# bobocode/lmono

Measured on AMD Instinct MI355X. Metric: KITTI HDL-64 scans/sec (scanRegistration + laserOdometry), higher is better.
Workload: dtype f32 features / f64 solve

## Files before the change

lmono_amd/csrc/batch.hpp:

```cpp
#pragma once
#include "common.hpp"

namespace lmono {

constexpr int kCornerTable = 16384;
constexpr int kSurfTable = 131072;
constexpr unsigned long long kEmptyKey = ~0ull;

struct __attribute__((aligned(16))) GridCell {
    unsigned long long key;
    int start;
    int cnt;
};

struct BatchView {
    const float4 *in;
    const int64_t *off;
    int n_scans;
    int scan0;
    int n_lines;
    int n_limit;
    int has_grid;
    float min_range;
    float4 *cloud;
    float *curv;
    int8_t *label;
    uint8_t *gap;
    int8_t *ring_tmp;
    int *seg_hist;
    int *scan_ends;
    int *scan_half;
    float *scan_ori;
    int *ring_begin;
    int *n_cloud;
    int *status;
    int *sel_sharp;
    int *sel_sharp_n;
    int *sel_flat;
    int *sel_flat_n;
    float4 *lf_tmp;
    int *lf_n;
    int *sel_todo;
    int *li_todo;
    int *vox_todo;
    float4 *sharp;
    float4 *less_sharp;
    float4 *flat;
    float4 *less_flat;
    int *feat_n;
    int *line_first_ge;
    int *line_last_le;
    GridCell *cg_cell;
    GridCell *sg_cell;
    float4 *cg_pts;
    float4 *sg_pts;
    float4 *lbc_pts;
    float4 *lbs_pts;
    int *lb_start;
    float4 *lb_elev;
    int *grid_mask;
};

}
```

lmono_amd/csrc/frontend.hip:

```cpp
#include "batch.hpp"
#include "ring_decide.hpp"
#include "sel_rounds.hpp"
#include "vox_runs.hpp"

namespace lmono {

__device__ __forceinline__ int ring_of(float angle, int n_lines, bool &discard)
{
    int id = 0;
    discard = false;
    if (n_lines == 16) {
        id = (int)((double)((angle + 15.0f) / 2.0f) + 0.5);
        if (id > n_lines - 1 || id < 0) discard = true;
    } else if (n_lines == 32) {
        id = (int)(((double)angle + 92.0 / 3.0) * 3.0 / 4.0);
        if (id > n_lines - 1 || id < 0) discard = true;
    } else {
        if ((double)angle >= -8.83)
            id = (int)((double)(2.0f - angle) * 3.0 + 0.5);
        else
            id = n_lines / 2 + (int)((-8.83 - (double)angle) * 2.0 + 0.5);
        if ((double)angle > 2.0 || (double)angle < -24.33 || id > 50 || id < 0) discard = true;
    }
    return id;
}

__device__ __forceinline__ bool point_valid(const float4 &p, float mr2)
{
    return isfinite(p.x) & isfinite(p.y) & isfinite(p.z) & !(p.x * p.x + p.y * p.y + p.z * p.z < mr2);
}

constexpr int kRtT = 256, kRtW = kRtT / 64;
constexpr int kRtSeg = 1024;
constexpr int kRtTile = kRtSeg * kRtW;

__device__ __forceinline__ int ring_scan_points(const BatchView &b, int s, int64_t off)
{
    const int n = (int)(b.off[s + 1] - off);
    return b.n_limit > 0 && b.n_limit < n ? b.n_limit : n;
}

__global__ __launch_bounds__(256) void k_ring_ends(BatchView b)
{
    const int s = b.scan0 + blockIdx.x;
    const int64_t off = b.off[s];
    const int n = ring_scan_points(b, s, off);
    const float4 *in = b.in + off;
    const int tid = threadIdx.x, lane = tid & 63;
    __shared__ int s_first;
    if (tid == 0) s_first = INT_MAX;
    __syncthreads();
    const float mr2 = b.min_range * b.min_range;
    for (int c0 = 0; c0 < n; c0 += 256) {
        const int i = c0 + tid;
        int lf = (i < n && point_valid(in[i], mr2)) ? i : INT_MAX;
        lf = wave_min_i(lf);
        if (lane == 0 && lf != INT_MAX) atomicMin(&s_first, lf);
        __syncthreads();
        const int f = s_first;
        __syncthreads();
        if (f != INT_MAX) break;
    }
    if (s_first == INT_MAX) {
        int *rb = b.ring_begin + s * 65;
        if (tid < 65) rb[tid] = 0;
        if (tid == 0) { b.n_cloud[s] = 0; b.scan_ends[s * 2] = -1; b.scan_ends[s * 2 + 1] = -1; b.scan_half[s] = INT_MAX; }
        return;
    }
    if (tid == 0) {
        const float4 p0 = in[s_first];
        b.scan_ori[s * 4] = (float)(-det_atan2((double)p0.y, (double)p0.x));
        float ux, uy;
        ring_start_dir(p0.x, p0.y, ux, uy);
        b.scan_ori[s * 4 + 2] = ux; b.scan_ori[s * 4 + 3] = uy;
        b.scan_ends[s * 2] = s_first; b.scan_ends[s * 2 + 1] = -1;
        b.scan_half[s] = INT_MAX;
    }
}

__global__ __launch_bounds__(kRtT) void k_ring_tag(BatchView b)
{
    const int s = b.scan0 + blockIdx.y;
    const int64_t off = b.off[s];
// ... 87 lines not shown
        for (int u = 0; u < 8; u++) t[u] = h[(size_t)(g + u) * 64];
#pragma unroll
        for (int u = 0; u < 8; u++) { h[(size_t)(g + u) * 64] = run; run += t[u]; }
    }
    for (; g < nseg; g++) { const int t = h[(size_t)g * 64]; h[(size_t)g * 64] = run; run += t; }
    int incl = run;
#pragma unroll
    for (int o = 1; o < 64; o <<= 1) { const int v = __shfl_up(incl, o); if (r >= o) incl += v; }
    int *rb = b.ring_begin + s * 65;
    rb[r] = incl - run;
    if (r == 63) { rb[64] = incl; b.n_cloud[s] = incl; }
}

__global__ __launch_bounds__(kRtT) void k_ring_scatter(BatchView b)
{
    const int s = b.scan0 + blockIdx.y;
    const int64_t off = b.off[s];
    const int n = ring_scan_points(b, s, off);
    const int t0 = blockIdx.x * kRtTile;
    if (t0 >= n || b.scan_ends[s * 2] < 0) return;
    const float4 *in = b.in + off;
    const int tid = threadIdx.x, lane = tid & 63, wave = tid >> 6;
    __shared__ int s_pos[kRtW][64];
    __shared__ double s_atan[17];
    if (tid < 17) s_atan[tid] = kAtanTab[tid];
    const int c_lo = t0 + wave * kRtSeg, c_hi = min(c_lo + kRtSeg, n);
    s_pos[wave][lane] = c_lo < n ? b.seg_hist[((size_t)(off >> 10) + (size_t)s + (size_t)(c_lo >> 10)) * 64 + lane] + b.ring_begin[s * 65 + lane] : 0;
    __syncthreads();
    const float startOri = b.scan_ori[s * 4], endOri = b.scan_ori[s * 4 + 1];
    const int half = b.scan_half[s];
    for (int r0 = c_lo; r0 < c_hi; r0 += 256) {
        int id[4], dstp[4];
        signed char idb[4];
#pragma unroll
        for (int q = 0; q < 4; q++) { const int i = r0 + 64 * q + lane; idb[q] = b.ring_tmp[off + min(i, c_hi - 1)]; }
#pragma unroll
        for (int q = 0; q < 4; q++) { const int i = r0 + 64 * q + lane; id[q] = (i < c_hi) ? (int)idb[q] : -1; }
        float4 pq[4];
#pragma unroll
        for (int q = 0; q < 4; q++) {
            const int i = r0 + 64 * q + lane;
            pq[q] = make_float4(0.f, 0.f, 0.f, 0.f);
            if (id[q] >= 0) pq[q] = in[i];
        }
#pragma unroll
        for (int q = 0; q < 4; q++) {
            dstp[q] = 0;
            unsigned long long rem = __ballot(id[q] >= 0);
            while (rem) {
                const int src = __ffsll((long long)rem) - 1;
                const int k = __shfl(id[q], src);
                const unsigned long long m = __ballot(id[q] == k);
                int base = 0;
                if (lane == src) { base = s_pos[wave][k]; s_pos[wave][k] = base + __popcll(m); }
                base = __shfl(base, src);
                if (id[q] == k) dstp[q] = base + __popcll(m & ((1ull << lane) - 1ull));
                rem &= ~m;
            }
        }
#pragma unroll
        for (int q = 0; q < 4; q++) {
            const int i = r0 + 64 * q + lane;
            if (id[q] >= 0) {
                const float4 p = pq[q];
                float ori = (float)(-det_atan2((double)p.y, (double)p.x, s_atan));
                if (i <= half) {
                    if ((double)ori < (double)startOri - LM_PI / 2.0) ori = (float)((double)ori + 2.0 * LM_PI);
                    else if ((double)ori > (double)startOri + LM_PI * 3.0 / 2.0) ori = (float)((double)ori - 2.0 * LM_PI);
                } else {
                    ori = (float)((double)ori + 2.0 * LM_PI);
                    if ((double)ori < (double)endOri - LM_PI * 3.0 / 2.0) ori = (float)((double)ori + 2.0 * LM_PI);
                    else if ((double)ori > (double)endOri + LM_PI / 2.0) ori = (float)((double)ori - 2.0 * LM_PI);
                }
                const float relTime = (ori - startOri) / (endOri - startOri);
                const float inten = (float)((double)id[q] + 0.1 * (double)relTime);
                b.cloud[off + dstp[q]] = make_float4(p.x, p.y, p.z, inten);
            }
        }
    }
}

constexpr int kCurvTile = 1024;

__global__ __launch_bounds__(256) void k_curvature(BatchView b)
{
    const int s = b.scan0 + blockIdx.y;
    const int n = b.n_cloud[s];
    const int t0 = blockIdx.x * kCurvTile;
    if (t0 >= n) return;
    const int64_t off = b.off[s];
    const float4 *c = b.cloud + off;
    __shared__ float sx[kCurvTile + 10], sy[kCurvTile + 10], sz[kCurvTile + 10];
    for (int k = threadIdx.x; k < kCurvTile + 10; k += 256) {
        const int i = t0 - 5 + k;
        float4 p = make_float4(0.f, 0.f, 0.f, 0.f);
        if (i >= 0 && i < n) p = c[i];
        sx[k] = p.x; sy[k] = p.y; sz[k] = p.z;
    }
    __syncthreads();
    for (int k = threadIdx.x; k < kCurvTile; k += 256) {
        const int i = t0 + k;
        if (i >= n) break;
        const int q = k + 5;
        float cv = 0.f;
        if (i >= 5 && i < n - 5) {
            const float dx = sx[q - 5] + sx[q - 4] + sx[q - 3] + sx[q - 2] + sx[q - 1] - 10 * sx[q] + sx[q + 1] + sx[q + 2] + sx[q + 3] + sx[q + 4] + sx[q + 5];
            const float dy = sy[q - 5] + sy[q - 4] + sy[q - 3] + sy[q - 2] + sy[q - 1] - 10 * sy[q] + sy[q + 1] + sy[q + 2] + sy[q + 3] + sy[q + 4] + sy[q + 5];
            const float dz = sz[q - 5] + sz[q - 4] + sz[q - 3] + sz[q - 2] + sz[q - 1] - 10 * sz[q] + sz[q + 1] + sz[q + 2] + sz[q + 3] + sz[q + 4] + sz[q + 5];
            cv = dx * dx + dy * dy + dz * dz;
        }
        b.curv[off + i] = cv;
        unsigned char g = 0;
        if (i + 1 < n) {
            const float gx = sx[q + 1] - sx[q], gy = sy[q + 1] - sy[q], gz = sz[q + 1] - sz[q];
            g = ((double)(gx * gx + gy * gy + gz * gz) > 0.05) ? 1 : 0;
        }
        b.gap[off + i] = g;
    }
}

constexpr int kSelMaxPerLane = (kRingCap / 6 + 1 + 63) / 64;

__device__ __forceinline__ unsigned int select_lo(int idx, unsigned int reach) { return ((unsigned int)idx << 8) | reach; }

__device__ __forceinline__ unsigned int lane_before(unsigned int v) { return (unsigned int)__builtin_amdgcn_update_dpp(0, (int)v, 0x138, 0xf, 0xf, true); }
__device__ __forceinline__ unsigned int lane_behind(unsigned int v) { return (unsigned int)__builtin_amdgcn_update_dpp(0, (int)v, 0x130, 0xf, 0xf, true); }

constexpr int kSelScratch = 64 * 8;

template <int M>
__device__ __forceinline__ void select_sector(int lane, int j, int sp, int slen, int rbeg, const float *curv, unsigned char *picked,
                                              signed char *label, const unsigned long long *gap, int *sel_sh, int *sel_sh_n, int *sel_fl, int *sel_fl_n,
                                              unsigned int *scratch)
{
    unsigned int kh[M], kl[M];
    unsigned int dead = 0, big = 0, small = 0;
    const int e0 = lane * M;
    unsigned int gwin;
    {
        const int jw = sp + min(e0, slen - 1) - 5;
        const unsigned long long wa = gap[jw >> 6], wb = gap[(jw >> 6) + 1];
        const int sh = jw & 63;
        gwin = (unsigned int)((wa >> sh) | (sh ? wb << (64 - sh) : 0ull));
    }
#pragma unroll
    for (int m = 0; m < M; m++) {
        const int e = e0 + m;
        const bool in = e < slen;
        const int i = sp + min(e, slen - 1);
        const float c = curv[i];
        const unsigned int win = gwin >> m;
        const int lf = min(5, __ffs((int)((win >> 5) | 32u)) - 1);
        const int lb = min(5, __clz((int)((win & 31u) << 27)));
        kh[m] = in ? __float_as_uint(c) : 0u; kl[m] = in ? select_lo(i, (unsigned int)(lf | (lb << 4))) : 0u;
        dead |= (unsigned int)(!in | (picked[i] != 0)) << m;
        big |= (unsigned int)(in & (c >= 0.1f)) << m;
        small |= (unsigned int)(in & (c < 0.1f)) << m;
    }
    int largest = 0;
    unsigned int members = 0u;
    {
        unsigned int live = big & ~dead;
        while (__ballot(live != 0u)) {
            unsigned int x[M + 2 * kSelReach];
#pragma unroll
            for (int m = 0; m < M; m++) x[m + kSelReach] = kh[m] & (unsigned int)((int)(live << (31 - m)) >> 31);
#pragma unroll
            for (int d = 0; d < kSelReach; d++) {
                x[d] = lane_before(x[M + d]);
                x[M + kSelReach + d] = lane_behind(x[kSelReach + d]);
            }
            const unsigned int w = sel_winners<M>(x, gwin);
            members |= w;
            live &= ~sel_deaths<M>(sel_window<M>(lane_before(w), w, lane_behind(w)), gwin);
        }
    }
    int n_mem = 0;
#pragma unroll
    for (int m = 0; m < M; m++) n_mem += __popcll(__ballot((members >> m) & 1u));
    unsigned int top = members;
    if (n_mem > 64) {
        const unsigned int best = sel_lane_best<M>(members, kh);
        int above = 0;
        for (int t = 0; t < 64; t++) above += (unsigned int)__builtin_amdgcn_readlane((int)best, t) > best ? 1 : 0;
        top = sel_keep_from<M>(members, kh, wave_min_u32_uniform(above < kSelSharpMax ? best : ~0u));
    }
    int n_top = 0;
#pragma unroll
    for (int m = 0; m < M; m++) {
        const bool is = (top >> m) & 1u;
        const unsigned long long mk = __ballot(is);
        const int pos = n_top + __popcll(mk & ((1ull << lane) - 1ull));
        if (is && pos < 64) { scratch[2 * pos] = kh[m]; scratch[2 * pos + 1] = kl[m]; }
        n_top += __popcll(mk);
    }
    const bool ranked = n_top <= 64;
    if (ranked) {
        __builtin_amdgcn_wave_barrier();
        unsigned int ch = 0u, cl = 0u;
        if (lane < n_top) { ch = scratch[2 * lane]; cl = scratch[2 * lane + 1]; }
        __builtin_amdgcn_wave_barrier();
        int rank = 0;
        for (int t = 0; t < n_top; t++) {
            const unsigned int th = (unsigned int)__builtin_amdgcn_readlane((int)ch, t), tl = (unsigned int)__builtin_amdgcn_readlane((int)cl, t);
            rank += sel_key_above(th, tl, ch, cl) ? 1 : 0;
        }
        if (lane < n_top && rank < kSelSharpMax) {
            const int pind = (int)(cl >> 8), lf = sel_lf(cl), lb = sel_lb(cl);
            sel_sh[j * 20 + rank] = rbeg + pind; label[pind] = rank < 2 ? 2 : 1;
#pragma unroll
            for (int o = 0; o <= 2 * kSelReach; o++) picked[pind - lb + min(o, lf + lb)] = 1;
        }
        largest = n_mem;
        __builtin_amdgcn_wave_barrier();
#pragma unroll
        for (int m = 0; m < M; m++) dead |= (unsigned int)(picked[sp + min(e0 + m, slen - 1)] != 0) << m;
    }
    while (!ranked) {
        const unsigned int live = big & ~dead;
        unsigned int bh = 0u, bl = 0u;
#pragma unroll
        for (int m = 0; m < M; m++) {
            const unsigned int h = kh[m] & (unsigned int)((int)(live << (31 - m)) >> 31);
            const bool t = h >= bh;
            bh = t ? h : bh; bl = t ? kl[m] : bl;
        }
        const unsigned int mh = wave_max_u32_uniform(bh);
        if (mh == 0u) break;
        const unsigned long long who = __ballot(bh == mh);
        unsigned int lo;
        if ((who & (who - 1ull)) == 0ull) lo = (unsigned int)__builtin_amdgcn_readlane((int)bl, __ffsll((long long)who) - 1);
        else lo = wave_max_u32_uniform(bh == mh ? bl : 0u);
        const int pind = (int)(lo >> 8), lf = (int)(lo & 15u), lb = (int)((lo >> 4) & 15u);
        largest++;
        if (largest > 20) break;
        if (lane == 0) { sel_sh[j * 20 + largest - 1] = rbeg + pind; label[pind] = largest <= 2 ? 2 : 1; }
        if (lane <= lf + lb) picked[pind - lb + lane] = 1;
        dead |= sel_hit_bits<M>(pind - lb - sp - e0, lb + lf);
    }
    if (lane == 0) sel_sh_n[j] = largest > 20 ? 20 : largest;
    int smallest = 0;
    while (true) {
        const unsigned int live = small & ~dead;
        unsigned int bh = ~0u, bl = ~0u;
#pragma unroll
        for (int m = 0; m < M; m++) {
            const unsigned int h = kh[m] | ~(unsigned int)((int)(live << (31 - m)) >> 31);
            const bool t = h < bh;
            bh = t ? h : bh; bl = t ? kl[m] : bl;
        }
        const unsigned int mh = wave_min_u32_uniform(bh);
        if (mh == ~0u) break;
        const unsigned long long who = __ballot(bh == mh);
        unsigned int lo;
        if ((who & (who - 1ull)) == 0ull) lo = (unsigned int)__builtin_amdgcn_readlane((int)bl, __ffsll((long long)who) - 1);
        else lo = wave_min_u32_uniform(bh == mh ? bl : ~0u);
        const int pind = (int)(lo >> 8), lf = (int)(lo & 15u), lb = (int)((lo >> 4) & 15u);
        if (lane == 0) { label[pind] = -1; sel_fl[j * 4 + smallest] = rbeg + pind; }
        smallest++;
        if (smallest >= 4) break;
        if (lane <= lf + lb) picked[pind - lb + lane] = 1;
        dead |= sel_hit_bits<M>(pind - lb - sp - e0, lb + lf);
    }
    if (lane == 0) sel_fl_n[j] = smallest;
}

__device__ __noinline__ void select_sector_wide(int lane, int j, int sp, int slen, int rbeg, const float *curv, unsigned char *picked,
                                                signed char *label, const unsigned long long *gap, int *sel_sh, int *sel_sh_n, int *sel_fl, int *sel_fl_n,
                                                unsigned int *scratch)
{
    select_sector<kSelMaxPerLane>(lane, j, sp, slen, rbeg, curv, picked, label, gap, sel_sh, sel_sh_n, sel_fl, sel_fl_n, scratch);
}

__device__ __forceinline__ int uni(int v) { return __builtin_amdgcn_readfirstlane(v); }
__device__ __forceinline__ long long uni64(long long v)
{
    const unsigned int lo = (unsigned int)__builtin_amdgcn_readfirstlane((int)(unsigned int)v), hi = (unsigned int)__builtin_amdgcn_readfirstlane((int)(unsigned int)((unsigned long long)v >> 32));
    return (long long)(((unsigned long long)hi << 32) | lo);
}
template <typename T> __device__ __forceinline__ T *uni_ptr(T *p)
{
    typedef __attribute__((address_space(1))) T GT;
    return (T *)(GT *)uni64((long long)p);
}

__host__ __device__ constexpr int sel_slice_bytes(int cap) { return 2 * cap; }

__device__ __forceinline__ void select_ring(BatchView &b, int r, int s, int lane, unsigned char *smem_w, int cap, bool may_defer, unsigned int *scratch)
{
    r = uni(r); s = uni(s);
    const int64_t off = uni64(b.off[s]);
    const int *rb = b.ring_begin + s * 65;
    const int rbeg = uni(rb[r]), rend = uni(rb[r + 1]), len = rend - rbeg;
    const int S = rbeg + 5, E = rend - 6;
    int *sel_sh = uni_ptr(b.sel_sharp + (size_t)((s * 64 + r) * kSectors) * 20);
    int *sel_sh_n = uni_ptr(b.sel_sharp_n + (s * 64 + r) * kSectors);
    int *sel_fl = uni_ptr(b.sel_flat + (size_t)((s * 64 + r) * kSectors) * 4);
    int *sel_fl_n = uni_ptr(b.sel_flat_n + (s * 64 + r) * kSectors);
    if (E - S < 6 || len > kRingCap) {
        if (lane < kSectors) { sel_sh_n[lane] = 0; sel_fl_n[lane] = 0; }
        if (lane == 0 && len > kRingCap) atomicOr(&b.status[s], kStatusRingOverflow);
        for (int i = lane; i < len; i += 64) b.label[off + rbeg + i] = 0;
        return;
    }
    if (len > cap) {
        if (may_defer && lane == 0) b.sel_todo[1 + atomicAdd(&b.sel_todo[0], 1)] = (s << 6) | r;
        return;
    }
    unsigned char *picked = smem_w;
    signed char *label = uni_ptr((signed char *)(b.label + off + rbeg));
    const float *curv = uni_ptr(b.curv + off + rbeg);
    const int span = E - S;
    unsigned long long *gap = (unsigned long long *)(picked + cap);
    for (int i0 = 0; i0 < len + 64; i0 += 64) {
        const int i = i0 + lane;
        unsigned char g = 0;
        if (i < len) { picked[i] = 0; label[i] = 0; g = b.gap[off + rbeg + i]; }
        const unsigned long long mk = __ballot(g != 0);
        if (lane == 0) gap[i0 >> 6] = mk;
    }
    __builtin_amdgcn_wave_barrier();
    for (int j = 0; j < kSectors; j++) {
        const int sp = 5 + span * j / 6;
        const int ep = 5 + span * (j + 1) / 6 - 1;
        const int slen = ep - sp + 1;
        if (slen <= 5 * 64) select_sector<5>(lane, j, sp, slen, rbeg, curv, picked, label, gap, sel_sh, sel_sh_n, sel_fl, sel_fl_n, scratch);
        else if (slen <= 6 * 64) select_sector<6>(lane, j, sp, slen, rbeg, curv, picked, label, gap, sel_sh, sel_sh_n, sel_fl, sel_fl_n, scratch);
        else select_sector_wide(lane, j, sp, slen, rbeg, curv, picked, label, gap, sel_sh, sel_sh_n, sel_fl, sel_fl_n, scratch);
    }
}

constexpr int kSelSmallCap = 2304, kSelBigGrid = 128;

__global__ __launch_bounds__(256, 8) void k_select(BatchView b, int cap, int from_list)
{
    const int lane = threadIdx.x & 63, wave = __builtin_amdgcn_readfirstlane((int)(threadIdx.x >> 6));
    extern __shared__ __align__(16) unsigned char smem[];
    unsigned char *smem_w = smem + wave * sel_slice_bytes(cap);
    unsigned int *scratch = (unsigned int *)(smem + 4 * sel_slice_bytes(cap) + wave * kSelScratch);
    if (!from_list) {
        select_ring(b, blockIdx.x * 4 + wave, b.scan0 + blockIdx.y, lane, smem_w, cap, true, scratch);
    } else {
        const int n_todo = b.sel_todo[0];
        for (int k = blockIdx.x * 4 + wave; k < n_todo; k += gridDim.x * 4) {
            const int e = b.sel_todo[1 + k];
            select_ring(b, e & 63, e >> 6, lane, smem_w, cap, false, scratch);
        }
    }
}

constexpr int kVoxBucketSegsBig = 1024;
constexpr int kVoxSmallSlots = 9, kVoxSmallBits = 11;
constexpr int kVoxBigSlots = kRingCap / 256, kVoxBigBits = 12;
constexpr int kVoxBigGrid = 512;
template <int kSlots, int kBits, bool kSmall>
struct VoxCfg {
    static constexpr int kSegCap = kSmall ? 256 * kSlots : kVoxBucketSegsBig;
    static constexpr int kHistBytes = (1 << kBits) * 2 > kSegCap * 2 ? (1 << kBits) * 2 : kSegCap * 2;
    static constexpr int kKeyBytes = kSmall ? kSegCap * 4 + kSegCap * 2 + kSegCap * 2 + kHistBytes : kRingCap * 8;
    static constexpr int kLds = kKeyBytes + 1024 + (kSlots * 4 + 2) * 8 + kSlots * 4 * 4;
};
static_assert(256 * kVoxSmallSlots <= 4096, "a first index of the small instantiation has 12 bits");
static_assert((1 << kVoxSmallBits) == 2048, "the small instantiation's counters are one uint4 per thread");
constexpr int kVoxLdsSmall = VoxCfg<kVoxSmallSlots, kVoxSmallBits, true>::kLds;
constexpr int kVoxLdsBig = VoxCfg<kVoxBigSlots, kVoxBigBits, false>::kLds;
static_assert(2 * kVoxBucketSegsBig * 8 + (1 << kVoxBigBits) * 4 <= kRingCap * 8, "bucket sort scratch must fit the key region");
#ifdef LMONO_VOX_PROF
#define VT(i) { if (blockIdx.x == 20 && blockIdx.y == 3 && threadIdx.x == 0) vt[i] = clock64(); }
#else
#define VT(i)
#endif

template <int kCtrl, int kRowMask>
__device__ __forceinline__ float dpp_mov_f32(float v, float ident)
{
    return __uint_as_float(dpp_mov_u32<kCtrl, kRowMask>(__float_as_uint(v), __float_as_uint(ident)));
}
__device__ __forceinline__ float wave_min_f(float v)
{
    v = fminf(v, dpp_mov_f32<0x111, 0xf>(v, FLT_MAX));
    v = fminf(v, dpp_mov_f32<0x112, 0xf>(v, FLT_MAX));
    v = fminf(v, dpp_mov_f32<0x114, 0xf>(v, FLT_MAX));
    v = fminf(v, dpp_mov_f32<0x118, 0xf>(v, FLT_MAX));
    v = fminf(v, dpp_mov_f32<0x142, 0xa>(v, FLT_MAX));
    v = fminf(v, dpp_mov_f32<0x143, 0xc>(v, FLT_MAX));
    return __uint_as_float((unsigned int)__builtin_amdgcn_readlane((int)__float_as_uint(v), 63));
}
__device__ __forceinline__ float wave_max_f(float v)
{
    v = fmaxf(v, dpp_mov_f32<0x111, 0xf>(v, -FLT_MAX));
    v = fmaxf(v, dpp_mov_f32<0x112, 0xf>(v, -FLT_MAX));
    v = fmaxf(v, dpp_mov_f32<0x114, 0xf>(v, -FLT_MAX));
    v = fmaxf(v, dpp_mov_f32<0x118, 0xf>(v, -FLT_MAX));
    v = fmaxf(v, dpp_mov_f32<0x142, 0xa>(v, -FLT_MAX));
    v = fmaxf(v, dpp_mov_f32<0x143, 0xc>(v, -FLT_MAX));
    return __uint_as_float((unsigned int)__builtin_amdgcn_readlane((int)__float_as_uint(v), 63));
}
__device__ __forceinline__ int wave_scan_incl_dpp(int v)
{
    v += (int)dpp_mov_u32<0x111, 0xf>((unsigned int)v, 0u);
    v += (int)dpp_mov_u32<0x112, 0xf>((unsigned int)v, 0u);
    v += (int)dpp_mov_u32<0x114, 0xf>((unsigned int)v, 0u);
    v += (int)dpp_mov_u32<0x118, 0xf>((unsigned int)v, 0u);
    v += (int)dpp_mov_u32<0x142, 0xa>((unsigned int)v, 0u);
    v += (int)dpp_mov_u32<0x143, 0xc>((unsigned int)v, 0u);
    return v;
}

template <int kVoxSlots, int kVoxBucketBits, bool kSmall>
__device__ __forceinline__ void voxel_ring(BatchView &b, int r, int s);

// ... 527 lines not shown
```

lmono_amd/csrc/lidar_abi.hip:

```cpp
#pragma once
constexpr int kListGrid = 256;

struct lmono_scan_batch {
    lmono_ctx *ctx = nullptr;
    int n_cap = 0;
    int64_t pts_cap = 0;
    int n_scans = 0;
    int64_t total = 0;
    int max_pts = 0;
    bool registered = false;
    bool grid_built = false;
    std::vector<int64_t> off_h;
    bool validation_pending = false;
    DevOwner mem;
    BatchView v{};
    int64_t *off_d = nullptr;
    float *in_owned = nullptr;
    hipEvent_t staged_ev = nullptr, in_free_ev = nullptr;
    int64_t staged_points = -1;
    std::vector<int> feat_h;
    int chains_cap = 0;
    double *state = nullptr, *incr = nullptr, *poses = nullptr, *xq = nullptr;
    int *corr = nullptr, *lm_info = nullptr, *corr_pair = nullptr, *seed = nullptr;
    float4 *crec = nullptr, *crec_pair = nullptr;
    float4 *lmrec = nullptr;
    size_t lmrec_cap = 0;
    unsigned int *wl = nullptr;
    size_t wl_cap = 0;
    double *ws = nullptr, *resid_d = nullptr;
    int *rstat = nullptr;
    unsigned int *rcount = nullptr;
    hipEvent_t rep_ev[2] = { nullptr, nullptr };
    lmono_boundary_report brep{};
    std::vector<double> resid_h;
    std::vector<int> rerun_h;
    int last_chains = 0, last_lead = 0, last_first = 0;
};

extern "C" void lmono_batch_destroy(lmono_scan_batch *b)
{
    if (!b) return;
    b->mem.clear();
    for (auto &e : b->rep_ev) if (e) (void)hipEventDestroy(e);
    if (b->staged_ev) (void)hipEventDestroy(b->staged_ev);
    if (b->in_free_ev) (void)hipEventDestroy(b->in_free_ev);
    delete b;
}

extern "C" lmono_scan_batch *lmono_batch_create(lmono_ctx *c, int n_cap, int64_t pts_cap)
{
    if (!c || n_cap <= 0 || pts_cap <= 0) return nullptr;
    if (hipSetDevice(c->device) != hipSuccess) return nullptr;
    lmono_scan_batch *b = new lmono_scan_batch();
    b->ctx = c; b->n_cap = n_cap; b->pts_cap = pts_cap;
    BatchView &v = b->v;
    const size_t T = (size_t)pts_cap, N = (size_t)n_cap;
    DevOwner &m = b->mem;
    bool ok = true;
    ok = ok && m.alloc(b->off_d, N + 1);
    ok = ok && m.alloc(v.cloud, T) && m.alloc(v.curv, T) && m.alloc(v.label, T) && m.alloc(v.gap, T);
    ok = ok && m.alloc(v.ring_tmp, T);
    ok = ok && m.alloc(v.seg_hist, ((T >> 10) + N + 1) * 64) && m.alloc(v.scan_ends, N * 2) && m.alloc(v.scan_half, N) && m.alloc(v.scan_ori, N * 4);
    ok = ok && m.alloc(v.ring_begin, N * 65) && m.alloc(v.n_cloud, N) && m.alloc(v.status, N);
    ok = ok && m.alloc(v.sel_sharp, N * 64 * 6 * 20) && m.alloc(v.sel_sharp_n, N * 64 * 6);
    ok = ok && m.alloc(v.sel_flat, N * 64 * 6 * 4) && m.alloc(v.sel_flat_n, N * 64 * 6);
    ok = ok && m.alloc(v.lf_tmp, T) && m.alloc(v.lf_n, N * 64) && m.alloc(v.vox_todo, N * 64 + 1) && m.alloc(v.sel_todo, N * 64 + 1) && m.alloc(v.li_todo, N * 2 + 1);
    ok = ok && m.alloc(v.sharp, N * kMaxSharp) && m.alloc(v.less_sharp, N * kMaxLessSharp);
    ok = ok && m.alloc(v.flat, N * kMaxFlat) && m.alloc(v.less_flat, T);
    ok = ok && m.alloc(v.feat_n, N * 4) && m.alloc(v.line_first_ge, N * 2 * 66) && m.alloc(v.line_last_le, N * 2 * 66);
    ok = ok && m.alloc(v.cg_cell, N * kCornerTable) && m.alloc(v.sg_cell, N * kSurfTable);
    ok = ok && m.alloc(v.cg_pts, N * kMaxLessSharp) && m.alloc(v.sg_pts, T) && m.alloc(v.grid_mask, N * 2);
    ok = ok && m.alloc(v.lbc_pts, N * kMaxLessSharp + kLbPad) && m.alloc(v.lbs_pts, T + kLbPad) && m.alloc(v.lb_start, N * 2 * (kLineKeys + 1)) && m.alloc(v.lb_elev, N * 2 * 66);
    ok = ok && m.alloc(b->incr, N * 7) && m.alloc(b->poses, N * 7) && m.alloc(b->xq, 8);
    ok = ok && m.alloc(b->corr_pair, (size_t)kMaxQueries * 4) && m.alloc(b->crec_pair, (size_t)kMaxQueries * 4);
    if (!ok) {
        c->err = "lmono_batch_create: hipMalloc failed";
        lmono_batch_destroy(b);
        return nullptr;
    }
    v.off = b->off_d;
    return b;
}

static int rings_used(int n_lines) { return n_lines == 64 ? 51 : n_lines; }

static int scanreg_launch(lmono_ctx *c, lmono_scan_batch *b, int scan0, int n_scans, int64_t max_pts, int n_limit = 0)
{
    BatchView v = b->v;
    v.scan0 = scan0; v.n_limit = n_limit;
    hipStream_t st = c->stream;
    c->ev = c->next_set();
    if (!c->ev) { c->err = "hipEventCreate failed"; return LMONO_ENODEV; }
    c->sets[c->n_sets - 1].reg = true;
    HIP_TRY(c, hipMemsetAsync(v.status + scan0, 0, sizeof(int) * n_scans, st));
    HIP_TRY(c, hipMemsetAsync(v.vox_todo, 0, sizeof(int), st));
    HIP_TRY(c, hipMemsetAsync(v.sel_todo, 0, sizeof(int), st));
    HIP_TRY(c, hipMemsetAsync(v.li_todo, 0, sizeof(int), st));
    HIP_TRY(c, hipEventRecord(c->ev[0], st));
    const int rt_tiles = (int)((max_pts + kRtTile - 1) / kRtTile);
    hipLaunchKernelGGL(k_ring_ends, dim3(n_scans), dim3(256), 0, st, v);
    if (rt_tiles > 0) hipLaunchKernelGGL(k_ring_tag, dim3(rt_tiles, n_scans), dim3(kRtT), 0, st, v);
    hipLaunchKernelGGL(k_ring_offsets, dim3(n_scans), dim3(64), 0, st, v);
    if (rt_tiles > 0) hipLaunchKernelGGL(k_ring_scatter, dim3(rt_tiles, n_scans), dim3(kRtT), 0, st, v);
    HIP_TRY(c, hipEventRecord(c->ev[1], st));
    const int tiles = (int)((max_pts + kCurvTile - 1) / kCurvTile);
    if (tiles > 0) hipLaunchKernelGGL(k_curvature, dim3(tiles, n_scans), dim3(256), 0, st, v);
    HIP_TRY(c, hipEventRecord(c->ev[2], st));
    const int n_rings = rings_used(b->v.n_lines);
    HIP_TRY(c, hipMemsetAsync(v.sel_sharp_n + (size_t)scan0 * 64 * 6, 0, sizeof(int) * (size_t)n_scans * 64 * 6, st));
    HIP_TRY(c, hipMemsetAsync(v.sel_flat_n + (size_t)scan0 * 64 * 6, 0, sizeof(int) * (size_t)n_scans * 64 * 6, st));
    HIP_TRY(c, hipMemsetAsync(v.lf_n + (size_t)scan0 * 64, 0, sizeof(int) * (size_t)n_scans * 64, st));
    hipLaunchKernelGGL(k_select, dim3((n_rings + 3) / 4, n_scans), dim3(256), 4 * sel_slice_bytes(kSelSmallCap) + 4 * kSelScratch, st, v, kSelSmallCap, 0);
    hipLaunchKernelGGL(k_select, dim3(kSelBigGrid), dim3(256), 4 * sel_slice_bytes(kRingCap) + 4 * kSelScratch, st, v, (int)kRingCap, 1);
    HIP_TRY(c, hipEventRecord(c->ev[3], st));
    hipLaunchKernelGGL((k_voxel<kVoxSmallSlots, kVoxSmallBits, true>), dim3(n_rings, n_scans), dim3(256), kVoxLdsSmall, st, v);
    hipLaunchKernelGGL((k_voxel<kVoxBigSlots, kVoxBigBits, false>), dim3(kVoxBigGrid), dim3(256), kVoxLdsBig, st, v);
    HIP_TRY(c, hipEventRecord(c->ev[4], st));
    hipLaunchKernelGGL(k_compact_index, dim3(n_scans), dim3(kLiT), kLiLdsHalf, st, v);
    HIP_TRY(c, hipEventRecord(c->ev[5], st));
#ifdef LMONO_DIAG_SEARCH
    if (c->opt[LMONO_OPT_CORR_TILE] != 3) {
        hipLaunchKernelGGL(k_grid_build, dim3(n_scans, 1 + kGridPar), dim3(1024), kGridLds, st, v);
        b->grid_built = true; v.has_grid = 1; b->v.has_grid = 1;
    }
#endif
    HIP_TRY(c, hipEventRecord(c->ev[6], st));
    hipLaunchKernelGGL(k_line_index<false>, dim3(kLiBigGrid), dim3(kLiT), kLiLdsFull, st, v);
    HIP_TRY(c, hipEventRecord(c->ev[7], st));
    return check_launch(c, "scanreg kernels");
}

extern "C" int lmono_scanreg_batch(lmono_ctx *c, lmono_scan_batch *b, const float *xyzi_d, const int64_t *offsets_h,
                                   int n_scans, int n_lines, float min_range);

static int batch_own_input(lmono_ctx *c, lmono_scan_batch *b)
{
    if (b->in_owned || b->mem.alloc(b->in_owned, (size_t)b->pts_cap * 4)) return LMONO_OK;
    const hipError_t e = hipGetLastError();
    c->err = std::string("hipMalloc(&q, (size_t)(b->pts_cap > 0 ? b->pts_cap : 1) * 16): ") + hipGetErrorString(e);
    return e == hipErrorOutOfMemory ? LMONO_ENOMEM : LMONO_ENODEV;
}

extern "C" int lmono_scanreg_batch_h(lmono_ctx *c, lmono_scan_batch *b, const float *xyzi_h, const int64_t *offsets_h,
                                     int n_scans, int n_lines, float min_range)
{
    if (!c || !b || !xyzi_h || !offsets_h || n_scans <= 0) return LMONO_EINVAL;
    if (offsets_h[0] != 0) { c->err = "offsets must start at 0"; return LMONO_EINVAL; }
    const int64_t total = offsets_h[n_scans];
    if (total < 0 || total > b->pts_cap) { c->err = "batch: too many points"; return LMONO_ECAPACITY; }
    HIP_TRY(c, hipSetDevice(c->device));
    if (int rc = batch_own_input(c, b)) return rc;
    if (total > 0) {
        HIP_TRY(c, hipMemcpyAsync(b->in_owned, xyzi_h, (size_t)total * 16, hipMemcpyHostToDevice, c->stream));
        HIP_TRY(c, hipStreamSynchronize(c->stream));
    }
    return lmono_scanreg_batch(c, b, b->in_owned, offsets_h, n_scans, n_lines, min_range);
}

extern "C" int lmono_scanreg_batch(lmono_ctx *c, lmono_scan_batch *b, const float *xyzi_d, const int64_t *offsets_h,
                                   int n_scans, int n_lines, float min_range)
{
    if (!c || !b || !xyzi_d || !offsets_h || n_scans <= 0) return LMONO_EINVAL;
    if (n_lines != 16 && n_lines != 32 && n_lines != 64) { c->err = "n_lines must be 16, 32 or 64"; return LMONO_EINVAL; }
    if (n_scans > b->n_cap) { c->err = "batch: too many scans"; return LMONO_ECAPACITY; }
    int64_t max_pts = 0;
    for (int s = 0; s < n_scans; s++) {
        const int64_t m = offsets_h[s + 1] - offsets_h[s];
        if (m < 0 || m > INT_MAX / 2) { c->err = "bad offsets"; return LMONO_EINVAL; }
        max_pts = m > max_pts ? m : max_pts;
    }
    const int64_t total = offsets_h[n_scans] - offsets_h[0];
    if (offsets_h[0] != 0) { c->err = "offsets must start at 0"; return LMONO_EINVAL; }
    if (total > b->pts_cap) { c->err = "batch: too many points"; return LMONO_ECAPACITY; }
    HIP_TRY(c, hipSetDevice(c->device));
    b->off_h.assign(offsets_h, offsets_h + n_scans + 1);
    b->n_scans = n_scans; b->total = total; b->max_pts = (int)max_pts; b->registered = false; b->grid_built = false;
    b->feat_h.clear();
    BatchView &v = b->v;
    v.in = (const float4 *)xyzi_d; v.n_scans = n_scans; v.scan0 = 0; v.n_lines = n_lines; v.min_range = min_range; v.has_grid = 0;
    HIP_TRY(c, hipMemcpyAsync(b->off_d, b->off_h.data(), sizeof(int64_t) * (n_scans + 1), hipMemcpyHostToDevice, c->stream));
    int rc = scanreg_launch(c, b, 0, n_scans, max_pts);
    if (rc) return rc;
    b->registered = true;
    return LMONO_OK;
}

extern "C" int lmono_batch_stage_h(lmono_ctx *c, lmono_scan_batch *b, const float *xyzi_h, int64_t total_points)
{
    if (!c || !b || !xyzi_h || total_points < 0) return LMONO_EINVAL;
// ... 33 lines not shown

extern "C" int lmono_timing_read(lmono_ctx *c, double *ms, int cap, int *n_scanreg_calls, int *n_odom_calls)
{
    if (!c || !ms) return LMONO_EINVAL;
    HIP_TRY(c, hipStreamSynchronize(c->stream));
    double sum[13] = { 0 };
    int nr = 0, no = 0;
    float t;
    for (int i = 0; i < c->n_sets; i++) {
        const EvSet &s = c->sets[i];
        if (s.reg) {
            nr++;
            if (hipEventElapsedTime(&t, s.e[0], s.e[7]) == hipSuccess) sum[0] += t;
            for (int k = 0; k < 7; k++)
                if (hipEventElapsedTime(&t, s.e[k], s.e[k + 1]) == hipSuccess) sum[2 + k] += t;
        }
        if (s.odom) {
            no++;
            if (hipEventElapsedTime(&t, s.e[8], s.e[9]) == hipSuccess) sum[1] += t;
            for (int k = 0; k + 2 < s.n_kev; k += 3) {
                if (k + 2 >= (int)s.kev.size()) break;
                if (hipEventElapsedTime(&t, s.kev[k], s.kev[k + 1]) == hipSuccess) sum[9] += t;
                if (hipEventElapsedTime(&t, s.kev[k + 1], s.kev[k + 2]) == hipSuccess) sum[10] += t;
                sum[11] += 1.0;
            }
        }
    }
    {
        unsigned long long st[40] = { 0 };
        HIP_TRY(c, hipMemcpy(st, c->stats_d, 320, hipMemcpyDeviceToHost));
        sum[12] = (double)st[0];
        for (int i = 1; i < 40 && 12 + i < cap; i++) ms[12 + i] = (double)st[i];
    }
    for (int i = 0; i < cap && i < 13; i++) ms[i] = sum[i];
    if (n_scanreg_calls) *n_scanreg_calls = nr;
    if (n_odom_calls) *n_odom_calls = no;
    return LMONO_OK;
}

extern "C" int lmono_batch_counts(lmono_ctx *c, lmono_scan_batch *b, int32_t *counts_h)
{
    if (!c || !b || !counts_h || !b->registered) return LMONO_EINVAL;
    const int n = b->n_scans;
    std::vector<int> nc(n), fn(n * 4), stt(n);
    HIP_TRY(c, hipStreamSynchronize(c->stream));
    HIP_TRY(c, hipMemcpy(nc.data(), b->v.n_cloud, sizeof(int) * n, hipMemcpyDeviceToHost));
    HIP_TRY(c, hipMemcpy(fn.data(), b->v.feat_n, sizeof(int) * n * 4, hipMemcpyDeviceToHost));
    HIP_TRY(c, hipMemcpy(stt.data(), b->v.status, sizeof(int) * n, hipMemcpyDeviceToHost));
    for (int s = 0; s < n; s++) {
        counts_h[6 * s] = nc[s];
        for (int k = 0; k < 4; k++) counts_h[6 * s + 1 + k] = fn[4 * s + k];
        counts_h[6 * s + 5] = stt[s];
    }
    return LMONO_OK;
}

extern "C" int lmono_batch_get_cloud(lmono_ctx *c, lmono_scan_batch *b, int scan, int which, float *out_h, int cap)
{
    if (!c || !b || !out_h || !b->registered || scan < 0 || scan >= b->n_scans || which < 0 || which > 4) return LMONO_EINVAL;
    HIP_TRY(c, hipStreamSynchronize(c->stream));
    int n = 0;
    const float4 *src = nullptr;
    int fn[4];
    HIP_TRY(c, hipMemcpy(fn, b->v.feat_n + scan * 4, sizeof(fn), hipMemcpyDeviceToHost));
    switch (which) {
    case 0: HIP_TRY(c, hipMemcpy(&n, b->v.n_cloud + scan, sizeof(int), hipMemcpyDeviceToHost)); src = b->v.cloud + b->off_h[scan]; break;
    case 1: n = fn[0]; src = b->v.sharp + (size_t)scan * kMaxSharp; break;
    case 2: n = fn[1]; src = b->v.less_sharp + (size_t)scan * kMaxLessSharp; break;
    case 3: n = fn[2]; src = b->v.flat + (size_t)scan * kMaxFlat; break;
    default: n = fn[3]; src = b->v.less_flat + b->off_h[scan]; break;
    }
    if (n > cap) { c->err = "get_cloud: output capacity too small"; return LMONO_ECAPACITY; }
    if (n > 0) HIP_TRY(c, hipMemcpy(out_h, src, sizeof(float4) * n, hipMemcpyDeviceToHost));
    return n;
}

extern "C" int lmono_batch_get_curvature(lmono_ctx *c, lmono_scan_batch *b, int scan, float *curv_h, int32_t *label_h, int cap)
{
    if (!c || !b || !b->registered || scan < 0 || scan >= b->n_scans) return LMONO_EINVAL;
    HIP_TRY(c, hipStreamSynchronize(c->stream));
    int n = 0;
    HIP_TRY(c, hipMemcpy(&n, b->v.n_cloud + scan, sizeof(int), hipMemcpyDeviceToHost));
    if (n > cap) { c->err = "get_curvature: output capacity too small"; return LMONO_ECAPACITY; }
    if (curv_h && n > 0) HIP_TRY(c, hipMemcpy(curv_h, b->v.curv + b->off_h[scan], sizeof(float) * n, hipMemcpyDeviceToHost));
    if (label_h && n > 0) {
        std::vector<int8_t> tmp(n);
        HIP_TRY(c, hipMemcpy(tmp.data(), b->v.label + b->off_h[scan], n, hipMemcpyDeviceToHost));
        for (int i = 0; i < n; i++) label_h[i] = tmp[i];
    }
    return n;
}

static int ensure_odom_ws(lmono_ctx *c, lmono_scan_batch *b, int n_chains)
{
    DevOwner &m = b->mem;
    const size_t lmrec_need = (size_t)(n_chains > b->chains_cap ? n_chains : b->chains_cap) * (4 - c->lm_planes) * kMaxQueries;
    if (lmrec_need > b->lmrec_cap) {
        if (!m.alloc(b->lmrec, lmrec_need)) { c->err = "odometry workspace: hipMalloc failed"; return LMONO_ENOMEM; }
        b->lmrec_cap = lmrec_need;
    }
    if (n_chains <= b->chains_cap) return LMONO_OK;
    bool ok = m.alloc(b->state, (size_t)n_chains * 8) && m.alloc(b->corr, (size_t)n_chains * kMaxQueries * 4) &&
              m.alloc(b->lm_info, (size_t)n_chains * 4) && m.alloc(b->crec, (size_t)n_chains * kMaxQueries * 4) &&
              m.alloc(b->seed, (size_t)n_chains * kMaxQueries) && m.alloc(b->wl, 8 * ((size_t)n_chains * kMaxQueries + 1)) &&
              m.alloc(b->ws, (size_t)n_chains * 8) && m.alloc(b->resid_d, (size_t)n_chains) && m.alloc(b->rstat, (size_t)n_chains * 4) &&
              m.alloc(b->rcount, (size_t)n_chains + 2);
    if (!ok) { c->err = "odometry workspace: hipMalloc failed"; return LMONO_ENOMEM; }
    b->chains_cap = n_chains;
    return LMONO_OK;
}

static int ensure_grid(lmono_ctx *c, lmono_scan_batch *b)
{
    if (b->grid_built) return LMONO_OK;
#ifdef LMONO_DIAG_SEARCH
    hipLaunchKernelGGL(k_grid_build, dim3(b->n_scans, 1 + kGridPar), dim3(1024), kGridLds, c->stream, b->v);
    int rc = check_launch(c, "k_grid_build");
    if (rc) return rc;
    b->grid_built = true; b->v.has_grid = 1;
    return LMONO_OK;
#else
    c->err = "the hash-grid searches exist in the diagnostic build only (-DLMONO_DIAG_SEARCH)";
    return LMONO_EINVAL;
#endif
}

struct GroupFork {
    lmono_ctx *c; int G, g_own; bool forked = false;
    GroupFork(lmono_ctx *c_, int G_, int g_own_) : c(c_), G(G_), g_own(g_own_) {}
    int fork()
    {
        if (G <= 1) return LMONO_OK;
        for (int g = g_own; g < G; g++)
            if (!c->gstream[g]) {
                int lo = 0, hi = 0;
                if (c->odom_prio && hipDeviceGetStreamPriorityRange(&lo, &hi) == hipSuccess) HIP_TRY(c, hipStreamCreateWithPriority(&c->gstream[g], hipStreamNonBlocking, hi));
                else HIP_TRY(c, hipStreamCreateWithFlags(&c->gstream[g], hipStreamNonBlocking));
            }
        for (int g = 0; g <= G && g < 9; g++) if (!c->gev[g]) HIP_TRY(c, hipEventCreateWithFlags(&c->gev[g], hipEventDisableTiming));
        HIP_TRY(c, hipEventRecord(c->gev[0], c->stream));
        forked = true;
        for (int g = g_own; g < G; g++) HIP_TRY(c, hipStreamWaitEvent(c->gstream[g], c->gev[0], 0));
        return LMONO_OK;
    }
    int join()
    {
        if (!forked) return LMONO_OK;
        forked = false;
        int rc = LMONO_OK;
        for (int g = g_own; g < G; g++) {
            if (hipEventRecord(c->gev[g + 1], c->gstream[g]) != hipSuccess || hipStreamWaitEvent(c->stream, c->gev[g + 1], 0) != hipSuccess) {
                (void)hipStreamSynchronize(c->gstream[g]);
                c->err = "odometry: joining a chain-group stream failed"; rc = LMONO_ENODEV;
            }
        }
        return rc;
    }
    ~GroupFork() { (void)join(); }
};

static int odom_groups(const lmono_ctx *c, int n_ch)
{
    constexpr int kMinChainsPerGroup = 32;
    int G = c->opt[LMONO_OPT_ODOM_STREAMS];
    G = G < 1 ? 1 : (G > 8 ? 8 : G);
    if (c->stream != nullptr && G > 3 && !c->many_queues) G = 3;
    while (G > 1 && n_ch / G < kMinChainsPerGroup) G--;
// ... 422 lines not shown
```

Before: 137,700.

## Fuse curvature and gap computation into selection kernel via DPP lane windows

Removes the separate curvature kernel and its curv/gap buffers from the hot path. The selection kernel now reads points directly and computes the curvature and gap-flag windows in registers, exchanging neighbour values between lanes with DPP shifts. Curvature is recomputed on demand only in the debug getter. This cuts a kernel launch and a global write plus re-read of curvature and gap data, at the cost of more register pressure and redundant point loads inside the selection kernel.

```diff
diff --git a/lmono_amd/csrc/batch.hpp b/lmono_amd/csrc/batch.hpp
--- a/lmono_amd/csrc/batch.hpp
+++ b/lmono_amd/csrc/batch.hpp
@@ -23,9 +23,7 @@
     int has_grid;
     float min_range;
     float4 *cloud;
-    float *curv;
     int8_t *label;
-    uint8_t *gap;
     int8_t *ring_tmp;
     int *seg_hist;
     int *scan_ends;
diff --git a/lmono_amd/csrc/curv_window.hpp b/lmono_amd/csrc/curv_window.hpp
--- /dev/null
+++ b/lmono_amd/csrc/curv_window.hpp
@@ -0,0 +1,75 @@
+#pragma once
+
+#if defined(__HIPCC__)
+#define LMONO_CW_HD __host__ __device__ __forceinline__
+#define LMONO_CW_UNROLL _Pragma("unroll")
+#else
+#define LMONO_CW_HD inline
+#define LMONO_CW_UNROLL
+#endif
+
+namespace lmono {
+
+constexpr int kCurvReach = 5;
+
+template <class T>
+LMONO_CW_HD T curv_diff(const T *w)
+{
+    return w[0] + w[1] + w[2] + w[3] + w[4] - 10 * w[5] + w[6] + w[7] + w[8] + w[9] + w[10];
+}
+
+LMONO_CW_HD bool curv_gap_long(float s) { return (double)s > 0.05; }
+LMONO_CW_HD unsigned int curv_gap_flag(float gx, float gy, float gz) { return curv_gap_long(gx * gx + gy * gy + gz * gz) ? 1u : 0u; }
+
+template <class U, class T>
+LMONO_CW_HD U curv_halo_flags(const T (&hx)[kCurvReach + 1], const T (&hy)[kCurvReach + 1], const T (&hz)[kCurvReach + 1])
+{
+    U hb = curv_gap_flag(hx[1] - hx[0], hy[1] - hy[0], hz[1] - hz[0]);
+    LMONO_CW_UNROLL
+    for (int d = 1; d < kCurvReach; d++) hb = hb | (curv_gap_flag(hx[d + 1] - hx[d], hy[d + 1] - hy[d], hz[d + 1] - hz[d]) << d);
+    return hb;
+}
+
+template <int M, class L, class T>
+LMONO_CW_HD typename L::bits curv_gap_window(const L &lanes, const T (&ox)[M], const T (&oy)[M], const T (&oz)[M],
+                                             const T &hx0, const T &hy0, const T &hz0, const typename L::bits &hb)
+{
+    static_assert(M >= kCurvReach, "one neighbour lane on either side must hold the five neighbours");
+    typedef typename L::bits U;
+    const T nx = lanes.behind(ox[0], hx0), ny = lanes.behind(oy[0], hy0), nz = lanes.behind(oz[0], hz0);
+    U own = curv_gap_flag(ox[1] - ox[0], oy[1] - oy[0], oz[1] - oz[0]);
+    LMONO_CW_UNROLL
+    for (int m = 1; m < M - 1; m++) own = own | (curv_gap_flag(ox[m + 1] - ox[m], oy[m + 1] - oy[m], oz[m + 1] - oz[m]) << m);
+    own = own | (curv_gap_flag(nx - ox[M - 1], ny - oy[M - 1], nz - oz[M - 1]) << (M - 1));
+    const U prev = lanes.before(own, hb << (M - kCurvReach));
+    const U next = lanes.behind(own, hb);
+    return (prev >> (M - kCurvReach)) | (own << kCurvReach) | (next << (M + kCurvReach));
+}
+
+template <int M, class T>
+LMONO_CW_HD void curv_window_accum(const T (&w)[M + 2 * kCurvReach], bool first, T (&cv)[M])
+{
+    LMONO_CW_UNROLL
+    for (int m = 0; m < M; m++) {
+        const T dc = curv_diff(w + m);
+        const T dd = dc * dc;
+        cv[m] = first ? dd : cv[m] + dd;
+    }
+}
+
+template <int M, class L, class T>
+LMONO_CW_HD void curv_window_coord(const L &lanes, const T (&own)[M], const T (&halo)[kCurvReach], bool first, T (&cv)[M])
+{
+    static_assert(M >= kCurvReach, "one neighbour lane on either side must hold the five neighbours");
+    T w[M + 2 * kCurvReach];
+    LMONO_CW_UNROLL
+    for (int m = 0; m < M; m++) w[m + kCurvReach] = own[m];
+    LMONO_CW_UNROLL
+    for (int d = 0; d < kCurvReach; d++) {
+        w[d] = lanes.before(own[M - kCurvReach + d], halo[d]);
+        w[M + kCurvReach + d] = lanes.behind(own[d], halo[d]);
+    }
+    curv_window_accum<M>(w, first, cv);
+}
+
+}
diff --git a/lmono_amd/csrc/frontend.hip b/lmono_amd/csrc/frontend.hip
--- a/lmono_amd/csrc/frontend.hip
+++ b/lmono_amd/csrc/frontend.hip
@@ -1,4 +1,5 @@
 #include "batch.hpp"
+#include "curv_window.hpp"
 #include "ring_decide.hpp"
 #include "sel_rounds.hpp"
 #include "vox_runs.hpp"
@@ -252,9 +253,8 @@
 
 constexpr int kCurvTile = 1024;
 
-__global__ __launch_bounds__(256) void k_curvature(BatchView b)
-{
-    const int s = b.scan0 + blockIdx.y;
+__global__ __launch_bounds__(256) void k_curvature(BatchView b, int s, float *curv)
+{
     const int n = b.n_cloud[s];
     const int t0 = blockIdx.x * kCurvTile;
     if (t0 >= n) return;
@@ -279,13 +279,7 @@
             const float dz = sz[q - 5] + sz[q - 4] + sz[q - 3] + sz[q - 2] + sz[q - 1] - 10 * sz[q] + sz[q + 1] + sz[q + 2] + sz[q + 3] + sz[q + 4] + sz[q + 5];
             cv = dx * dx + dy * dy + dz * dz;
         }
-        b.curv[off + i] = cv;
-        unsigned char g = 0;
-        if (i + 1 < n) {
-            const float gx = sx[q + 1] - sx[q], gy = sy[q + 1] - sy[q], gz = sz[q + 1] - sz[q];
-            g = ((double)(gx * gx + gy * gy + gz * gz) > 0.05) ? 1 : 0;
-        }
-        b.gap[off + i] = g;
+        curv[i] = cv;
     }
 }
 
@@ -298,27 +292,72 @@
 
 constexpr int kSelScratch = 64 * 8;
 
+struct SelLanes {
+    typedef unsigned int bits;
+    __device__ __forceinline__ unsigned int before(unsigned int v, unsigned int old) const { return (unsigned int)__builtin_amdgcn_update_dpp((int)old, (int)v, 0x138, 0xf, 0xf, false); }
+    __device__ __forceinline__ unsigned int behind(unsigned int v, unsigned int old) const { return (unsigned int)__builtin_amdgcn_update_dpp((int)old, (int)v, 0x130, 0xf, 0xf, false); }
+    __device__ __forceinline__ float before(float v, float old) const { return __uint_as_float(before(__float_as_uint(v), __float_as_uint(old))); }
+    __device__ __forceinline__ float behind(float v, float old) const { return __uint_as_float(behind(__float_as_uint(v), __float_as_uint(old))); }
+};
+
 template <int M>
-__device__ __forceinline__ void select_sector(int lane, int j, int sp, int slen, int rbeg, const float *curv, unsigned char *picked,
-                                              signed char *label, const unsigned long long *gap, int *sel_sh, int *sel_sh_n, int *sel_fl, int *sel_fl_n,
+__device__ __forceinline__ void select_sector(int lane, int j, int sp, int slen, int rbeg, const float4 *pts, unsigned char *picked,
+                                              signed char *label, int *sel_sh, int *sel_sh_n, int *sel_fl, int *sel_fl_n,
                                               unsigned int *scratch)
 {
     unsigned int kh[M], kl[M];
     unsigned int dead = 0, big = 0, small = 0;
+    asm volatile("" : "+v"(lane));
     const int e0 = lane * M;
+    float cv[M];
     unsigned int gwin;
     {
-        const int jw = sp + min(e0, slen - 1) - 5;
-        const unsigned long long wa = gap[jw >> 6], wb = gap[(jw >> 6) + 1];
-        const int sh = jw & 63;
-        gwin = (unsigned int)((wa >> sh) | (sh ? wb << (64 - sh) : 0ull));
+        const int last = slen + 4;
+        const float4 *hp = pts + sp + (lane == 0 ? -kCurvReach : min(64 * M, last));
+        const int hmax = lane == 0 ? kCurvReach : max(last - 64 * M, 0);
+        const SelLanes lanes;
+        unsigned int hb;
+        float hx0, hy0, hz0;
+        {
+            float h[3][kCurvReach + 1];
+#pragma unroll
+            for (int d = 0; d <= kCurvReach; d++) {
+                const float4 p = hp[min(d, hmax)];
+                h[0][d] = p.x; h[1][d] = p.y; h[2][d] = p.z;
+            }
+            hb = curv_halo_flags<unsigned int>(h[0], h[1], h[2]);
+            hx0 = h[0][0]; hy0 = h[1][0]; hz0 = h[2][0];
+        }
+        float o[3][M];
+#pragma unroll
+        for (int m = 0; m < M; m++) {
+            const float4 p = pts[sp + min(e0 + m, last)];
+            o[0][m] = p.x; o[1][m] = p.y; o[2][m] = p.z;
+        }
+        gwin = curv_gap_window<M>(lanes, o[0], o[1], o[2], hx0, hy0, hz0, hb);
+#pragma unroll
+        for (int c = 0; c < 3; c++) {
+            float h[kCurvReach];
+#pragma unroll
+            for (int d = 0; d < kCurvReach; d++) h[d] = ((const float *)(hp + min(d, hmax)))[c];
+            if constexpr (M <= 6) {
+                curv_window_coord<M>(lanes, o[c], h, c == 0, cv);
+            } else {
+                float oc[M];
+                int ec = e0;
+                asm volatile("" : "+v"(ec));
+#pragma unroll
+                for (int m = 0; m < M; m++) oc[m] = ((const float *)(pts + sp + min(ec + m, last)))[c];
+                curv_window_coord<M>(lanes, oc, h, c == 0, cv);
+            }
+        }
     }
 #pragma unroll
     for (int m = 0; m < M; m++) {
         const int e = e0 + m;
         const bool in = e < slen;
         const int i = sp + min(e, slen - 1);
-        const float c = curv[i];
+        const float c = cv[m];
         const unsigned int win = gwin >> m;
         const int lf = min(5, __ffs((int)((win >> 5) | 32u)) - 1);
         const int lb = min(5, __clz((int)((win & 31u) << 27)));
@@ -435,11 +474,11 @@
     if (lane == 0) sel_fl_n[j] = smallest;
 }
 
-__device__ __noinline__ void select_sector_wide(int lane, int j, int sp, int slen, int rbeg, const float *curv, unsigned char *picked,
-                                                signed char *label, const unsigned long long *gap, int *sel_sh, int *sel_sh_n, int *sel_fl, int *sel_fl_n,
+__device__ __noinline__ void select_sector_wide(int lane, int j, int sp, int slen, int rbeg, const float4 *pts, unsigned char *picked,
+                                                signed char *label, int *sel_sh, int *sel_sh_n, int *sel_fl, int *sel_fl_n,
                                                 unsigned int *scratch)
 {
-    select_sector<kSelMaxPerLane>(lane, j, sp, slen, rbeg, curv, picked, label, gap, sel_sh, sel_sh_n, sel_fl, sel_fl_n, scratch);
+    select_sector<kSelMaxPerLane>(lane, j, sp, slen, rbeg, pts, picked, label, sel_sh, sel_sh_n, sel_fl, sel_fl_n, scratch);
 }
 
 __device__ __forceinline__ int uni(int v) { return __builtin_amdgcn_readfirstlane(v); }
@@ -479,24 +518,18 @@
     }
     unsigned char *picked = smem_w;
     signed char *label = uni_ptr((signed char *)(b.label + off + rbeg));
-    const float *curv = uni_ptr(b.curv + off + rbeg);
+    const float4 *pts = uni_ptr((const float4 *)(b.cloud + off + rbeg));
     const int span = E - S;
-    unsigned long long *gap = (unsigned long long *)(picked + cap);
-    for (int i0 = 0; i0 < len + 64; i0 += 64) {
-        const int i = i0 + lane;
-        unsigned char g = 0;
-        if (i < len) { picked[i] = 0; label[i] = 0; g = b.gap[off + rbeg + i]; }
-        const unsigned long long mk = __ballot(g != 0);
-        if (lane == 0) gap[i0 >> 6] = mk;
-    }
+#pragma unroll 1
+    for (int i = lane; i < len; i += 64) { picked[i] = 0; label[i] = 0; }
     __builtin_amdgcn_wave_barrier();
     for (int j = 0; j < kSectors; j++) {
         const int sp = 5 + span * j / 6;
         const int ep = 5 + span * (j + 1) / 6 - 1;
         const int slen = ep - sp + 1;
-        if (slen <= 5 * 64) select_sector<5>(lane, j, sp, slen, rbeg, curv, picked, label, gap, sel_sh, sel_sh_n, sel_fl, sel_fl_n, scratch);
-        else if (slen <= 6 * 64) select_sector<6>(lane, j, sp, slen, rbeg, curv, picked, label, gap, sel_sh, sel_sh_n, sel_fl, sel_fl_n, scratch);
-        else select_sector_wide(lane, j, sp, slen, rbeg, curv, picked, label, gap, sel_sh, sel_sh_n, sel_fl, sel_fl_n, scratch);
+        if (slen <= 5 * 64) select_sector<5>(lane, j, sp, slen, rbeg, pts, picked, label, sel_sh, sel_sh_n, sel_fl, sel_fl_n, scratch);
+        else if (slen <= 6 * 64) select_sector<6>(lane, j, sp, slen, rbeg, pts, picked, label, sel_sh, sel_sh_n, sel_fl, sel_fl_n, scratch);
+        else select_sector_wide(lane, j, sp, slen, rbeg, pts, picked, label, sel_sh, sel_sh_n, sel_fl, sel_fl_n, scratch);
     }
 }
 
diff --git a/lmono_amd/csrc/lidar_abi.hip b/lmono_amd/csrc/lidar_abi.hip
--- a/lmono_amd/csrc/lidar_abi.hip
+++ b/lmono_amd/csrc/lidar_abi.hip
@@ -19,6 +19,8 @@
     hipEvent_t staged_ev = nullptr, in_free_ev = nullptr;
     int64_t staged_points = -1;
     std::vector<int> feat_h;
+    float *curv = nullptr;
+    size_t curv_cap = 0;
     int chains_cap = 0;
     double *state = nullptr, *incr = nullptr, *poses = nullptr, *xq = nullptr;
     int *corr = nullptr, *lm_info = nullptr, *corr_pair = nullptr, *seed = nullptr;
@@ -58,7 +60,7 @@
     DevOwner &m = b->mem;
     bool ok = true;
     ok = ok && m.alloc(b->off_d, N + 1);
-    ok = ok && m.alloc(v.cloud, T) && m.alloc(v.curv, T) && m.alloc(v.label, T) && m.alloc(v.gap, T);
+    ok = ok && m.alloc(v.cloud, T) && m.alloc(v.label, T);
     ok = ok && m.alloc(v.ring_tmp, T);
     ok = ok && m.alloc(v.seg_hist, ((T >> 10) + N + 1) * 64) && m.alloc(v.scan_ends, N * 2) && m.alloc(v.scan_half, N) && m.alloc(v.scan_ori, N * 4);
     ok = ok && m.alloc(v.ring_begin, N * 65) && m.alloc(v.n_cloud, N) && m.alloc(v.status, N);
@@ -103,8 +105,6 @@
     hipLaunchKernelGGL(k_ring_offsets, dim3(n_scans), dim3(64), 0, st, v);
     if (rt_tiles > 0) hipLaunchKernelGGL(k_ring_scatter, dim3(rt_tiles, n_scans), dim3(kRtT), 0, st, v);
     HIP_TRY(c, hipEventRecord(c->ev[1], st));
-    const int tiles = (int)((max_pts + kCurvTile - 1) / kCurvTile);
-    if (tiles > 0) hipLaunchKernelGGL(k_curvature, dim3(tiles, n_scans), dim3(256), 0, st, v);
     HIP_TRY(c, hipEventRecord(c->ev[2], st));
     const int n_rings = rings_used(b->v.n_lines);
     HIP_TRY(c, hipMemsetAsync(v.sel_sharp_n + (size_t)scan0 * 64 * 6, 0, sizeof(int) * (size_t)n_scans * 64 * 6, st));
@@ -304,7 +304,13 @@
     int n = 0;
     HIP_TRY(c, hipMemcpy(&n, b->v.n_cloud + scan, sizeof(int), hipMemcpyDeviceToHost));
     if (n > cap) { c->err = "get_curvature: output capacity too small"; return LMONO_ECAPACITY; }
-    if (curv_h && n > 0) HIP_TRY(c, hipMemcpy(curv_h, b->v.curv + b->off_h[scan], sizeof(float) * n, hipMemcpyDeviceToHost));
+    if (curv_h && n > 0) {
+        if (!b->mem.grow_replace(b->curv, b->curv_cap, (size_t)n, 1 << 17)) { c->err = "get_curvature: hipMalloc failed"; return LMONO_ENOMEM; }
+        hipLaunchKernelGGL(k_curvature, dim3((n + kCurvTile - 1) / kCurvTile), dim3(256), 0, c->stream, b->v, scan, b->curv);
+        if (int rc = check_launch(c, "k_curvature")) return rc;
+        HIP_TRY(c, hipMemcpyAsync(curv_h, b->curv, sizeof(float) * n, hipMemcpyDeviceToHost, c->stream));
+        HIP_TRY(c, hipStreamSynchronize(c->stream));
+    }
     if (label_h && n > 0) {
         std::vector<int8_t> tmp(n);
         HIP_TRY(c, hipMemcpy(tmp.data(), b->v.label + b->off_h[scan], n, hipMemcpyDeviceToHost));
```

Result: faster. 141,400, median of 6 (+2.7%).
